# haoheliu/AudioLDM2

Measured on NVIDIA H100. Metric: 10s clips/sec @200 DDIM steps (audioldm2-full), higher is better.
Workload: dtype f16x2 (split-fp16 tensor-core operands: weights hi + lo, activations hi + lo in the convolutions and one plane on the token side; fp32 accumulate, fp32 residual stream)

## Files before the change

### audioldm2_b200/_lib.py

```python
from __future__ import annotations

import ctypes as C
import os
import shutil
import subprocess
import sys

HERE = os.path.dirname(os.path.abspath(__file__))
ROOT = os.path.dirname(HERE)
CSRC = os.path.join(HERE, "csrc")
LIB_PATH = os.path.join(HERE, "libaldm_b200.so")
SOURCES = ["gemm.cu", "prep.cu", "attention.cu", "elementwise.cu", "stft.cu", "program.cu", "engine_abi.cu", "microbench.cu",
           "cond/seqgen.cu"]
NVCC_FLAGS = ["-gencode", "arch=compute_90a,code=sm_90a", "-lineinfo", "-O3", "-std=c++17",
              "-Xcompiler", "-fPIC", "--use_fast_math=false"]

NVCC = shutil.which("nvcc") or os.path.join(os.environ.get("CUDA_HOME", "/usr/local/cuda"), "bin", "nvcc")

MAX_TAPS = 16
ABI_VERSION = 9

GEMM_TC, GEMM_SIMT, GEMM_TC_V1 = 0, 1, 2
GEMM_STATIC_B = 1 << 16
ACT_NONE, ACT_GEGLU, ACT_TANH, ACT_SILU, ACT_GELU_TANH = 0, 1, 2, 3, 4
OUT_F32, OUT_PLANES, OUT_NCHW, OUT_QKV = 0, 1, 2, 3
EPI_FAST, EPI_GEGLU, EPI_GENERIC, EPI_F32N, EPI_PLN = 0, 1, 2, 3, 4
RED_NONE, RED_REDUCE4, RED_GENERIC = 0, 1, 2
STORE_ROW, STORE_COMPACT, STORE_PAIR_PLN, STORE_PAIR_GEGLU, STORE_PAIR_QK = 0, 1, 2, 3, 4
PREP_COPY, PREP_SILU, PREP_LRELU, PREP_GN, PREP_GN_SILU, PREP_LN = 0, 1, 2, 3, 4, 5
OP_GEMM, OP_PREP, OP_ATTN, OP_SOFTMAX, OP_TEMB, OP_TRANSPOSE, OP_PACKB, OP_COPY = 1, 2, 3, 4, 5, 6, 7, 8
OP_SEQ_ASSEMBLE, OP_KV_ATTN, OP_SEQ_FEEDBACK = 9, 10, 11


class GemmDesc(C.Structure):
    _fields_ = [
        ("a_hi", C.c_void_p), ("a_lo", C.c_void_p), ("w_packed", C.c_void_p), ("w_plain", C.c_void_p),
        ("bias", C.c_void_p), ("rowvec", C.c_void_p), ("res", C.c_void_p), ("out", C.c_void_p),
        ("out_hi", C.c_void_p), ("out_lo", C.c_void_p), ("out2_hi", C.c_void_p), ("out2_lo", C.c_void_p),
        ("ws", C.c_void_p),
        ("B", C.c_int32), ("H", C.c_int32), ("W", C.c_int32), ("Cp", C.c_int32),
        ("up", C.c_int32), ("bmod", C.c_int32),
        ("OH", C.c_int32), ("OW", C.c_int32), ("sy", C.c_int32), ("sx", C.c_int32),
        ("ntaps", C.c_int32),
        ("dy", C.c_int16 * MAX_TAPS), ("dx", C.c_int16 * MAX_TAPS),
        ("N", C.c_int32), ("K", C.c_int32), ("Kpad", C.c_int32), ("bn", C.c_int32),
        ("ldo", C.c_int32), ("ld_res", C.c_int32), ("ld_rowvec", C.c_int32),
        ("OHF", C.c_int32), ("OWF", C.c_int32), ("osy", C.c_int32), ("ooy", C.c_int32),
        ("act", C.c_int32), ("out_mode", C.c_int32), ("accumulate", C.c_int32), ("splitk", C.c_int32),
        ("impl", C.c_int32), ("n_split", C.c_int32), ("tok_per_batch", C.c_int32), ("ld_t", C.c_int32),
        ("alpha", C.c_float),
    ]


class PrepDesc(C.Structure):
    _fields_ = [
        ("src0", C.c_void_p), ("src1", C.c_void_p), ("gamma", C.c_void_p), ("beta", C.c_void_p),
        ("out_hi", C.c_void_p), ("out_lo", C.c_void_p), ("scratch", C.c_void_p),
        ("rows", C.c_int32), ("c0", C.c_int32), ("c1", C.c_int32), ("Cp", C.c_int32),
        ("B", C.c_int32), ("HW", C.c_int32), ("groups", C.c_int32), ("mode", C.c_int32),
        ("eps", C.c_float), ("slope", C.c_float), ("src_nchw", C.c_int32),
    ]
# ... 93 lines not shown
        objs.append(o)
        cmd = [NVCC] + [f for f in NVCC_FLAGS if not f.startswith("--use_fast_math")] + ["-c", s, "-o", o]
        if verbose:
            print(" ".join(cmd))
        procs.append((cmd, subprocess.Popen(cmd, stdout=subprocess.PIPE, stderr=subprocess.STDOUT)))
    for cmd, p in procs:
        out, _ = p.communicate()
        if p.returncode != 0:
            raise RuntimeError("nvcc failed: %s\n%s" % (" ".join(cmd), out.decode()))
        if verbose and out:
            print(out.decode())
    cmd = [NVCC, "-shared", "-o", LIB_PATH] + objs + ["-lcudart"]
    r = subprocess.run(cmd, stdout=subprocess.PIPE, stderr=subprocess.STDOUT)
    if r.returncode != 0:
        raise RuntimeError("link failed: %s\n%s" % (" ".join(cmd), r.stdout.decode()))
    return LIB_PATH


_lib = None


def lib() -> C.CDLL:
    global _lib
    if _lib is not None:
        return _lib
    if not os.path.exists(LIB_PATH):
        raise RuntimeError(f"{LIB_PATH} is missing: run `python -c 'import __graft_entry__ as g; g.build()'`. "
                           "There is no CPU/PyTorch fallback for the native path.")
    L = C.CDLL(LIB_PATH)
    vp, i32, i64, f32 = C.c_void_p, C.c_int32, C.c_int64, C.c_float
    sig = {
        "aldm_gemm": (i32, [C.POINTER(GemmDesc), vp]),
        "aldm_gemm_variant": (i32, [C.POINTER(GemmDesc), C.POINTER(i32)]),
        "aldm_prep": (i32, [C.POINTER(PrepDesc), vp]),
        "aldm_pack_b": (i32, [vp, i32, i32, i32, i32, i32, vp, vp, vp]),
        "aldm_attention": (i32, [C.POINTER(AttnDesc), vp]),
        "aldm_kv_attention": (i32, [C.POINTER(KvAttnDesc), vp]),
        "aldm_seq_assemble": (i32, [C.POINTER(SeqAssembleDesc), vp]),
        "aldm_seq_feedback": (i32, [C.POINTER(SeqFeedbackDesc), vp]),
        "aldm_softmax_rows": (i32, [vp, i32, i32, f32, vp, vp, vp]),
        "aldm_timestep_embedding": (i32, [vp, i32, i32, vp, vp, vp, vp]),
        "aldm_ddim_step": (i32, [vp, vp, vp, vp, vp, vp, i64, f32, f32, f32, f32, f32, vp]),
        "aldm_masked_blend": (i32, [vp, vp, vp, vp, i32, i32, i32, f32, f32, vp]),
        "aldm_transpose_chw": (i32, [vp, vp, i32, i32, i32, i32, vp]),
        "aldm_posterior_sample": (i32, [vp, vp, vp, i32, i32, i32, f32, vp]),
        "aldm_stft_mel": (i32, [vp, i32, i32, i32, i32, vp, i32, vp, i32, vp]),
        "aldm_program_create": (i32, [C.POINTER(Op), i32, C.POINTER(vp)]),
        "aldm_program_run": (i32, [vp, vp]),
        "aldm_program_run_range": (i32, [vp, i32, i32, vp]),
        "aldm_program_capture": (i32, [vp, vp]),
        "aldm_program_replay": (i32, [vp, vp]),
        "aldm_program_num_launches": (i32, [vp]),
        "aldm_program_is_captured": (i32, [vp]),
        "aldm_program_destroy": (None, [vp]),
        "aldm_engine_create": (i32, [C.POINTER(EngineDesc), C.POINTER(vp)]),
        "aldm_engine_destroy": (None, [vp]),
        "aldm_engine_set_conditioning": (i32, [vp, i32, vp, vp, i32, vp, vp, i32, vp, vp]),
        "aldm_engine_precompute": (i32, [vp, vp]),
        "aldm_engine_unet_eps": (i32, [vp, vp, i64, vp, vp, vp]),
        "aldm_engine_ddim_step": (i32, [vp, vp, i64, vp, f32, f32, f32, f32, f32, vp, vp, vp]),
        "aldm_engine_vae_decode": (i32, [vp, vp, vp, vp]),
        "aldm_engine_vocoder": (i32, [vp, vp, vp, vp]),
        "aldm_engine_vae_encode": (i32, [vp, vp, vp, vp]),
        "aldm_sizeof_engine_desc": (C.c_size_t, []),
        "aldm_abi_version": (i32, []),
        "aldm_sizeof_op": (C.c_size_t, []),
        "aldm_sizeof_gemm_desc": (C.c_size_t, []),
        "aldm_offsetof_gemm": (C.c_size_t, [i32]),
        "aldm_last_error": (C.c_char_p, []),
        "aldm_device_check": (i32, [i32]),
        "aldm_debug_timeline": (i32, [vp, i32]),
        "aldm_debug_store_rate": (i32, [i32, i32, i32, i64, vp]),
    }
    for name, (res, args) in sig.items():
        fn = getattr(L, name)
        fn.restype = res
        fn.argtypes = args
    if L.aldm_abi_version() != ABI_VERSION:
        raise RuntimeError("libaldm_b200.so ABI version mismatch: rebuild")
    if L.aldm_sizeof_engine_desc() != C.sizeof(EngineDesc):
        raise RuntimeError("ctypes mirror of aldm_engine_desc does not match the C layout")
    if L.aldm_sizeof_op() != C.sizeof(Op) or L.aldm_sizeof_gemm_desc() != C.sizeof(GemmDesc):
        raise RuntimeError("ctypes mirror of aldm_op / aldm_gemm_desc does not match the C layout")
    _lib = L
    return L


EXPORTED = ["aldm_gemm", "aldm_gemm_variant", "aldm_prep", "aldm_pack_b", "aldm_attention", "aldm_softmax_rows",
            "aldm_kv_attention", "aldm_seq_assemble", "aldm_seq_feedback",
            "aldm_timestep_embedding", "aldm_ddim_step", "aldm_masked_blend", "aldm_transpose_chw",
            "aldm_posterior_sample", "aldm_stft_mel", "aldm_program_create", "aldm_program_run",
            "aldm_program_run_range", "aldm_program_capture", "aldm_program_replay",
            "aldm_program_num_launches", "aldm_program_is_captured", "aldm_program_destroy", "aldm_engine_create",
            "aldm_engine_destroy", "aldm_engine_set_conditioning", "aldm_engine_precompute", "aldm_engine_unet_eps",
            "aldm_engine_ddim_step", "aldm_engine_vae_decode", "aldm_engine_vocoder", "aldm_engine_vae_encode",
            "aldm_sizeof_engine_desc", "aldm_abi_version", "aldm_sizeof_op",
            "aldm_sizeof_gemm_desc", "aldm_offsetof_gemm", "aldm_last_error", "aldm_device_check", "aldm_debug_timeline",
            "aldm_debug_store_rate"]


def gemm_variant(d: GemmDesc) -> tuple:
    out = (C.c_int32 * 5)()
    check(lib().aldm_gemm_variant(C.byref(d), out), "gemm_variant")
    return tuple(out)


def check(rc: int, what: str = ""):
    if rc != 0:
        msg = lib().aldm_last_error().decode(errors="replace")
        raise RuntimeError(f"aldm error {rc} {what}: {msg}")


if __name__ == "__main__":
    print(build(verbose="-v" in sys.argv, force="-f" in sys.argv))
```

### audioldm2_b200/csrc/gemm.cu

```cuda
#include <stdlib.h>

#include "common.cuh"

namespace aldm {

struct RowInfo {
  int m, b, oh, ow;
  bool valid;
  long long orow;
};

__device__ __forceinline__ RowInfo decode_row(const aldm_gemm_desc& d, int m, int M) {
  RowInfo r;
  r.m = m;
  r.valid = m < M;
  int mm = r.valid ? m : 0;
  r.ow = mm % d.OW;
  int t = mm / d.OW;
  r.oh = t % d.OH;
  r.b = t / d.OH;
  r.orow = ((long long)r.b * d.OHF + (long long)r.oh * d.osy + d.ooy) * d.OWF + r.ow;
  return r;
}

// ... 203 lines not shown
    const auto o = cr.orow[it] * d.ldo + n;
    if (!PLANES_ONLY) *reinterpret_cast<float4*>(d.out + o) = x;
    if (PLANES_ONLY || d.out_hi) {
      uint2 h, l;
      split2(x.x, x.y, h.x, l.x);
      split2(x.z, x.w, h.y, l.y);
      *reinterpret_cast<uint2*>(reinterpret_cast<aldm_plane_t*>(d.out_hi) + o) = h;
      if (d.out_lo) *reinterpret_cast<uint2*>(reinterpret_cast<aldm_plane_t*>(d.out_lo) + o) = l;
    }
  }
  __syncwarp();
}

__device__ __forceinline__ void line_put_hi(uint8_t* tile, int lane, int part, const float* v) {
  uint8_t* wr = tile + lane * 128;
  const int sw = lane & 7;
#pragma unroll
  for (int j = 0; j < 4; ++j) *reinterpret_cast<uint4*>(wr + (((part * 4 + j) ^ sw) << 4)) = pack8_hi(v + 8 * j);
}
template <typename CR>
__device__ __forceinline__ void line_store_hi(const aldm_gemm_desc& d, const CR& cr, int n_group0, const uint8_t* tile, int lane) {
  __syncwarp();
  const int rs = lane >> 3, c8 = lane & 7;
  aldm_plane_t* out = reinterpret_cast<aldm_plane_t*>(d.out_hi);
#pragma unroll
  for (int it = 0; it < 8; ++it) {
    const int rr = it * 4 + rs;
    const uint4 x = *reinterpret_cast<const uint4*>(tile + rr * 128 + ((c8 ^ (rr & 7)) << 4));
    if ((cr.vmask >> rr) & 1u) *reinterpret_cast<uint4*>(out + (cr.orow[it] * d.ldo + n_group0 + c8 * 8)) = x;
  }
  __syncwarp();
}

template <int BN, int AP>
struct Tc3Cfg {
  static constexpr int BM = 128;
  static constexpr int BK = 64;
  static constexpr int A_BYTES = BM * 128;
  static constexpr int B_BYTES = BN * 128;
  static constexpr int STAGE_BYTES = AP * A_BYTES + 2 * B_BYTES;
  static constexpr int B_OFF = AP * A_BYTES;
  static constexpr int ACC_BYTES = BM * BN * 4;
  static constexpr int STG_BYTES = 4 * 32 * 33 * 4;
  static constexpr int SMEM_MAX = 227 * 1024;
  static constexpr int FIT = (SMEM_MAX - 1024 - 256 - STG_BYTES - ACC_BYTES) / STAGE_BYTES;
  static constexpr int STAGES = FIT > 4 ? 4 : FIT;
  static constexpr int SMEM_BYTES = STAGES * STAGE_BYTES + ACC_BYTES + 1024  + 256  + STG_BYTES;
  static_assert(STAGES >= 2, "pipeline needs two stages");
  static_assert(SMEM_BYTES <= SMEM_MAX, "shared memory");
};

template <int BN>
__device__ __forceinline__ void acc_st_frag(float* accb, int row0, int lane, const float* d) {
  const int g = lane >> 2, t = lane & 3;
#pragma unroll
  for (int h = 0; h < 2; ++h) {
    const int row = row0 + g + 8 * h;
    float* rp = accb + row * BN + 2 * (t & 1);
#pragma unroll
    for (int j = 0; j < BN / 8; ++j)
      *reinterpret_cast<float2*>(rp + (((2 * j + (t >> 1)) ^ (row & 7)) << 2)) = make_float2(d[4 * j + 2 * h], d[4 * j + 2 * h + 1]);
  }
}
template <int BN>
__device__ __forceinline__ void acc_ld32(const float* accb, int row, int c0, uint32_t* r) {
  const float* rp = accb + row * BN;
#pragma unroll
  for (int j = 0; j < 8; ++j) {
    const float4 x = *reinterpret_cast<const float4*>(rp + ((((c0 >> 2) + j) ^ (row & 7)) << 2));
    r[4 * j] = __float_as_uint(x.x); r[4 * j + 1] = __float_as_uint(x.y);
    r[4 * j + 2] = __float_as_uint(x.z); r[4 * j + 3] = __float_as_uint(x.w);
  }
}
constexpr int kProdRegs = 80, kConsRegs = 136, kEpiRegs = 160;
static_assert(kProdRegs + 2 * kConsRegs + kEpiRegs == 4 * 128, "register split must use exactly the launch allocation");
template <int R>
__device__ __forceinline__ void setmaxnreg_dec() { asm volatile("setmaxnreg.dec.sync.aligned.u32 %0;" ::"n"(R)); }
template <int R>
__device__ __forceinline__ void setmaxnreg_inc() { asm volatile("setmaxnreg.inc.sync.aligned.u32 %0;" ::"n"(R)); }

__device__ long long g_timeline[4 * 256 * 2];
#define ALDM_TL(role, i, ph)                                                      \
  do {                                                                            \
    if ((dbg & 128) && blockIdx.x == 0 && (i) < 256) g_timeline[((role) * 256 + (i)) * 2 + (ph)] = clock64(); \
  } while (0)

enum { EPI_FAST = ALDM_EPI_FAST, EPI_GEGLU = ALDM_EPI_GEGLU, EPI_GENERIC = ALDM_EPI_GENERIC, EPI_F32N = ALDM_EPI_F32N,
       EPI_PLN = ALDM_EPI_PLN };

struct FastDiv {
  unsigned long long M;
  int sh;
  int d;
  __device__ __forceinline__ int div(int n) const {
    return (int)(((unsigned long long)(unsigned)n * M) >> sh);
  }
  __device__ __forceinline__ void divmod(int n, int& q, int& r) const { q = div(n); r = n - q * d; }
};
static FastDiv make_fastdiv(int d) {
  FastDiv f;
  int l = 0;
  while ((1ll << l) < d) ++l;
  f.M = (unsigned long long)((((unsigned __int128)1) << (32 + l)) / (unsigned)d) + 1ull;
  f.sh = 32 + l;
  f.d = d;
  if (d == 1) { f.M = 1ull << 32; f.sh = 32; }
  return f;
}
struct Tc3Divs {
  FastDiv ow, oh, cp, tn, bmod;
  int plain;
  int store;
};

template <int BN, int EPI, int AP>
__global__ void __launch_bounds__(512, 1) gemm_tc3_kernel(const __grid_constant__ aldm_gemm_desc d, int tiles_m, int tiles_n,
                                                           const __grid_constant__ Tc3Divs fd) {
  using C = Tc3Cfg<BN, AP>;
  extern __shared__ uint8_t smem_raw[];
  const uint32_t raw = smem_u32(smem_raw);
  const uint32_t base = (raw + 1023u) & ~1023u;
  const uint32_t acc_base = base + C::STAGES * C::STAGE_BYTES;
  const uint32_t bar_base = acc_base + C::ACC_BYTES;
  auto full_bar = [&](int s) { return bar_base + 8u * s; };
  auto empty_bar = [&](int s) { return bar_base + 8u * (C::STAGES + s); };
  const uint32_t acc_full = bar_base + 8u * (2 * C::STAGES);
  const uint32_t acc_empty = acc_full + 8u;
  float* accb = reinterpret_cast<float*>(smem_raw + (acc_base - raw));

  const int tid = threadIdx.x;
  const int warp = tid >> 5;
  const int lane = tid & 31;
  const int M = d.B * d.OH * d.OW;
  const int nkb_total = d.Kpad / C::BK;
  const int total = tiles_m * tiles_n * d.splitk;
  const int dbg = d.impl >> 8;

  if (tid == 0) {
    for (int s = 0; s < C::STAGES; ++s) {
      mbar_init(full_bar(s), 128 + 1);
      mbar_init(empty_bar(s), 8);
    }
    mbar_init(acc_full, 8);
    mbar_init(acc_empty, 4);
    fence_barrier_init();
  }
  __syncthreads();

  auto tile_coords = [&](int id, int& mt, int& nt, int& z, int& kb0, int& nkb) {
    int r = id;
    z = 0; kb0 = 0; nkb = nkb_total;
    if (d.splitk > 1) {
      z = id % d.splitk;
      r = id / d.splitk;
      kb0 = (int)(((long long)z * nkb_total) / d.splitk);
      nkb = (int)(((long long)(z + 1) * nkb_total) / d.splitk) - kb0;
    }
    fd.tn.divmod(r, mt, nt);
  };

  if (warp >= 8 && warp < 12) {
    setmaxnreg_dec<kProdRegs>();
    const int ptid = tid - 256;
    const int j = ptid & 7;
    const int rbase = ptid >> 3;
    const uint32_t swz = (uint32_t)((j ^ (rbase & 7)) << 4);
    const int Hs = d.H >> d.up, Ws = d.W >> d.up;
    const aldm_plane_t* ahi = reinterpret_cast<const aldm_plane_t*>(d.a_hi);
    const aldm_plane_t* alo = reinterpret_cast<const aldm_plane_t*>(d.a_lo);
    uint32_t cnt = 0;
    int last_mt = -1;
    int rowoff[8];
    uint32_t tapmask[8];
    uint32_t yx0[8];
    auto decode_rows = [&](int mt) {
#pragma unroll
      for (int i = 0; i < 8; ++i) {
        const int m = mt * C::BM + rbase + 16 * i;
        uint32_t msk = 0, yx = 0;
        int off = 0;
        if (fd.plain) {
          if (m < M) { msk = 16u; off = m * d.Cp; }
        } else if (m < M) {
          int t, ow, b, oh;
          fd.ow.divmod(m, t, ow);
          fd.oh.divmod(t, b, oh);
          const int y0 = oh * d.sy, x0 = ow * d.sx;
          int bs = b;
          if (d.bmod > 0) { int q; fd.bmod.divmod(b, q, bs); }
          const int pb = bs * Hs;
          yx = (uint32_t)y0 | ((uint32_t)x0 << 16);
          for (int tp = 0; tp < d.ntaps; ++tp) {
            const int ih = y0 + d.dy[tp], iw = x0 + d.dx[tp];
            if (ih >= 0 && ih < d.H && iw >= 0 && iw < d.W) msk |= 16u << tp;
          }
// ... 69 lines not shown
          if (!(dbg & 1)) {
#define ALDM_A_ROW(i)                                                                            \
            {                                                                                      \
              const uint32_t nb = (tapmask[i] >> sh) & 16u;                                        \
              cp_async_16_off<(i) * 2048>(sa2, ab + rowoff[i], nb);                                \
              if (AP == 2) cp_async_16_off<(i) * 2048 + C::A_BYTES>(sa2, abl + rowoff[i], nb);     \
            }
            ALDM_A_ROW(0) ALDM_A_ROW(1) ALDM_A_ROW(2) ALDM_A_ROW(3) ALDM_A_ROW(4) ALDM_A_ROW(5) ALDM_A_ROW(6) ALDM_A_ROW(7)
#undef ALDM_A_ROW
          }
        } else {
          const int dy = d.dy[tp], dx = d.dx[tp];
#pragma unroll
          for (int i = 0; i < 8; ++i) {
            const bool ok = kvalid && ((tapmask[i] >> (tp + 4)) & 1u);
            long long off = 0;
            const int ih = (int)(yx0[i] & 0xffffu) + dy, iw = (int)(yx0[i] >> 16) + dx;
            if (ok) off = ((long long)(rowoff[i] + (ih >> 1)) * Ws + (iw >> 1)) * d.Cp + c;
            const uint32_t dst = sa + (uint32_t)(rbase + 16 * i) * 128u;
            cp_async_16(dst, ahi + off, ok ? 16u : 0u);
            if (AP == 2) cp_async_16(dst + C::A_BYTES, alo + off, ok ? 16u : 0u);
          }
        }
        cp_async_mbar_arrive_noinc(full_bar(s));
        if (ptid == 0) ALDM_TL(0, cnt, 1);
        c += C::BK;
        while (c >= d.Cp) { c -= d.Cp; ++tap; }
      }
    }
  } else if (warp < 8) {
    setmaxnreg_inc<kConsRegs>();
    pdl_wait();
    const int wg = warp >> 2;
    uint32_t cnt = 0, tl = 0;
    float acc[BN / 2];
    for (int id = blockIdx.x; id < total; id += gridDim.x, ++tl) {
      int mt, nt, z, kb0, nkb;
      tile_coords(id, mt, nt, z, kb0, nkb);
#pragma unroll
      for (int i = 0; i < BN / 2; ++i) acc[i] = 0.f;
      for (int it = 0; it < nkb; ++it, ++cnt) {
        const int s = cnt % C::STAGES;
        if (it > 0) {
          wgmma_wait<0>();
          if (lane == 0) mbar_arrive(empty_bar((cnt - 1) % C::STAGES));
        }
        mbar_wait(full_bar(s), (cnt / C::STAGES) & 1);
        if (tid == 0) ALDM_TL(2, cnt, 0);
        fence_proxy_async();
        const uint32_t sa = base + s * C::STAGE_BYTES;
        const uint64_t da_hi = wgmma_desc_sw128(sa + wg * 64 * 128);
        const uint64_t da_lo = wgmma_desc_sw128(sa + C::A_BYTES + wg * 64 * 128);
        const uint64_t db_hi = wgmma_desc_sw128(sa + C::B_OFF);
        const uint64_t db_lo = wgmma_desc_sw128(sa + C::B_OFF + C::B_BYTES);
        wgmma_fence();
        if (!(dbg & 4)) {
#pragma unroll
          for (int ks = 0; ks < 4; ++ks) {
            const uint64_t o = (uint64_t)(ks * 2);
            wgmma_ss<BN>(acc, da_hi + o, db_lo + o, 1);
            if (AP == 2) wgmma_ss<BN>(acc, da_lo + o, db_hi + o, 1);
            wgmma_ss<BN>(acc, da_hi + o, db_hi + o, 1);
          }
        }
        wgmma_commit();
        if (tid == 0) ALDM_TL(2, cnt, 1);
      }
      wgmma_wait<0>();
      wgmma_fence_regs<BN / 2>(acc);
      if (lane == 0) mbar_arrive(empty_bar((cnt - 1) % C::STAGES));
      if (tid == 0 && id + (int)gridDim.x >= total) pdl_launch();
      mbar_wait(acc_empty, (tl & 1) ^ 1);
      acc_st_frag<BN>(accb, wg * 64 + (warp & 3) * 16, lane, acc);
      __syncwarp();
      if (lane == 0) mbar_arrive(acc_full);
    }
  } else {
    setmaxnreg_inc<kEpiRegs>();
    pdl_wait();
    const int ew = warp - 12;
    const int trow_in_tile = ew * 32 + lane;
    float* stg = reinterpret_cast<float*>(smem_raw + (bar_base + 256 - raw)) + ew * (32 * 33);
    uint8_t* stg8 = reinterpret_cast<uint8_t*>(stg);
    constexpr bool kCompact = EPI == EPI_F32N || EPI == EPI_PLN;
    constexpr int NCH = BN / 32;
    constexpr int NRV = NCH > 1 ? 2 : 1;
    constexpr int NGV = BN >= 64 ? BN / 64 : 1;
    const bool pair_pln = EPI == EPI_PLN && BN >= 64 && fd.store == ALDM_STORE_PAIR_PLN;
    const bool pair_geglu = EPI == EPI_GEGLU && BN == 128 && fd.store == ALDM_STORE_PAIR_GEGLU;
    const bool pair_qk = EPI == EPI_FAST && BN >= 64 && fd.store == ALDM_STORE_PAIR_QK;
    const bool has_res = kCompact && d.res != nullptr;
    uint32_t tl = 0;
    for (int id = blockIdx.x; id < total; id += gridDim.x, ++tl) {
      int mt, nt, z, kb0, nkb;
      tile_coords(id, mt, nt, z, kb0, nkb);
      const int m = mt * C::BM + trow_in_tile;
      RowInfo r;
      {
        r.m = m; r.valid = m < M;
        const int mm = r.valid ? m : 0;
        int t;
        fd.ow.divmod(mm, t, r.ow);
        fd.oh.divmod(t, r.b, r.oh);
        r.orow = ((long long)r.b * d.OHF + (long long)r.oh * d.osy + d.ooy) * d.OWF + r.ow;
      }
      CoRows cr;
      CoRows32 cr32;
      if (kCompact) cr32 = co_rows32(r, lane); else cr = co_rows(r, lane);
      float4 pb4[NCH], prv[NRV][8];
      if (kCompact) {
#pragma unroll
        for (int ch = 0; ch < NCH; ++ch) {
          const int n = nt * BN + 32 * ch + (lane & 7) * 4;
          pb4[ch] = (d.bias && n < d.N) ? __ldg(reinterpret_cast<const float4*>(d.bias + n)) : make_float4(0.f, 0.f, 0.f, 0.f);
        }
#pragma unroll
        for (int ch = 0; ch < NRV; ++ch)
          if (has_res) co_load_res32(d, cr32, nt * BN + 32 * ch, d.N, lane, prv[ch]);
      }
      float pln_b[NCH];
#pragma unroll
      for (int ch = 0; ch < NCH; ++ch) {
        const int n = nt * BN + 32 * ch + lane;
        pln_b[ch] = (pair_pln && d.bias && n < d.N) ? __ldg(d.bias + n) : 0.f;
      }
      float gb_v[NGV], gb_g[NGV];
#pragma unroll
      for (int c = 0; c < NGV; ++c) {
        gb_v[c] = 0.f; gb_g[c] = 0.f;
        if (EPI == EPI_GEGLU && d.bias && d.splitk == 1) {
          gb_v[c] = __ldg(d.bias + nt * BN + 32 * c + lane);
// ... 239 lines not shown
      pc0 = tile * d.bn + sub * 32; n0 = tile * (d.bn / 2) + sub * 32; n_out = d.N / 2;
    } else {
      pc0 = ch * 32; n0 = pc0; n_out = d.N;
    }
    const float* wv = d.w_plain + (long long)(pc0 + lane) * d.Kpad;
    const float* wg = wv + (long long)(d.bn / 2) * d.Kpad;
    float acc = 0.f, accg = 0.f;
    for (int tap = 0; tap < d.ntaps; ++tap) {
      const int ih = r.oh * d.sy + d.dy[tap], iw = r.ow * d.sx + d.dx[tap];
      if (ih < 0 || ih >= d.H || iw < 0 || iw >= d.W) continue;
      const long long off = ((long long)(bsrc * Hs + (ih >> d.up)) * Ws + (iw >> d.up)) * d.Cp;
      const float* wt = wv + tap * d.Cp;
      const float* wgt = wg + tap * d.Cp;
      for (int c = 0; c < d.Cp; ++c) {
        const float a = plane_to_f(ahi[off + c]) + (alo ? plane_to_f(alo[off + c]) : 0.f);
        acc = fmaf(a, __ldg(wt + c), acc);
        if (geglu) accg = fmaf(a, __ldg(wgt + c), accg);
      }
    }
    float v[32], g[32];
#pragma unroll
    for (int i = 0; i < 32; ++i) {
      v[i] = __shfl_sync(0xffffffffu, acc, i);
      g[i] = __shfl_sync(0xffffffffu, accg, i);
    }
    if (lane == 0) {
      epi_activate(d, r, pc0, v, g);
      epi_finish(d, r, n0, 32, v, n_out);
    }
  }
}

struct GemmVariant {
  int bn, epi, ap, red, store;
};

static GemmVariant gemm_select(const aldm_gemm_desc& d) {
  GemmVariant v{d.bn, EPI_GENERIC, d.a_lo ? 2 : 1, ALDM_RED_NONE, ALDM_STORE_ROW};
  const int BN = d.bn;
  const bool geglu = d.act == ALDM_ACT_GEGLU;
  const int n_out = geglu ? d.N / 2 : d.N;
  const bool co = d.splitk == 1 && n_out % 4 == 0 && d.ldo % 4 == 0 && (!d.res || d.ld_res % 4 == 0) &&
                  (d.out_mode == ALDM_OUT_F32 || d.out_mode == ALDM_OUT_PLANES || d.out_mode == ALDM_OUT_QKV);
  const long long out_rows = (long long)d.B * d.OHF * d.OWF;
  const int ld_max = d.ldo > d.ld_res ? d.ldo : d.ld_res;
  static const bool compact_on = [] { const char* e = getenv("ALDM_EPI_COMPACT"); return !(e && e[0] == '0'); }();
  const bool plain = compact_on && co && d.act == ALDM_ACT_NONE && d.alpha == 1.0f && !d.accumulate && !d.rowvec &&
                     out_rows * ld_max < (1ll << 31) &&
                     (!d.bias || aligned16(d.bias)) && (!d.res || aligned16(d.res));
  if (co && geglu && !d.res && d.out_mode != ALDM_OUT_QKV && BN >= 64) v.epi = EPI_GEGLU;
  else if (plain && d.out_mode == ALDM_OUT_F32 && aligned16(d.out) && (!d.out_hi || d.ldo % 4 == 0)) v.epi = EPI_F32N;
  else if (plain && d.out_mode == ALDM_OUT_PLANES) v.epi = EPI_PLN;
  else if (co && d.act == ALDM_ACT_NONE) v.epi = EPI_FAST;
  if (v.epi == EPI_F32N || v.epi == EPI_PLN) v.store = ALDM_STORE_COMPACT;
  const bool pair_ok = d.out_lo == nullptr && d.splitk == 1 && d.ldo % 8 == 0 && aligned16(d.out_hi);
  if (v.epi == EPI_PLN && BN >= 64 && pair_ok && d.res == nullptr && d.N % BN == 0) v.store = ALDM_STORE_PAIR_PLN;
  if (v.epi == EPI_GEGLU && BN == 128 && pair_ok && d.out_mode == ALDM_OUT_PLANES && (d.N / 2) % 64 == 0) v.store = ALDM_STORE_PAIR_GEGLU;
  if (v.epi == EPI_FAST && BN >= 64 && pair_ok && d.out_mode == ALDM_OUT_QKV && d.res == nullptr && d.n_split % 64 == 0)
    v.store = ALDM_STORE_PAIR_QK;
  if (d.splitk > 1) {
    const bool fast = d.act == ALDM_ACT_NONE && d.alpha == 1.0f && !d.accumulate && d.N % 4 == 0 && d.ldo % 4 == 0 &&
                      (d.out_mode == ALDM_OUT_F32 || d.out_mode == ALDM_OUT_PLANES) && (!d.res || (d.ld_res % 4 == 0 && aligned16(d.res))) &&
                      (!d.bias || aligned16(d.bias)) && (!d.rowvec || (d.ld_rowvec % 4 == 0 && aligned16(d.rowvec))) &&
                      (d.out_mode != ALDM_OUT_F32 || aligned16(d.out));
    v.red = fast ? ALDM_RED_REDUCE4 : ALDM_RED_GENERIC;
  }
  return v;
}

template <int BN, int EPI, int AP>
static int launch_tc3_ap(const aldm_gemm_desc& d, int M, const GemmVariant& v, cudaStream_t st) {
  using C = Tc3Cfg<BN, AP>;
  static bool configured = false;
  if (!configured) {
    ALDM_CHECK_CUDA(cudaFuncSetAttribute(gemm_tc3_kernel<BN, EPI, AP>, cudaFuncAttributeMaxDynamicSharedMemorySize, C::SMEM_BYTES));
    configured = true;
  }
  const int tiles_m = cdiv(M, C::BM), tiles_n = cdiv(d.N, BN);
  const long long total = (long long)tiles_m * tiles_n * d.splitk;
  const int grid = (int)(total < num_sms() ? total : num_sms());
  Tc3Divs fd;
  fd.ow = make_fastdiv(d.OW); fd.oh = make_fastdiv(d.OH); fd.cp = make_fastdiv(d.Cp); fd.tn = make_fastdiv(tiles_n);
  fd.bmod = make_fastdiv(d.bmod > 0 ? d.bmod : 1);
  fd.plain = d.ntaps == 1 && d.dy[0] == 0 && d.dx[0] == 0 && d.sy == 1 && d.sx == 1 && d.up == 0 && d.bmod <= 0 &&
             d.OH == d.H && d.OW == d.W;
  fd.store = v.store;
  ALDM_CHECK_CUDA(launch_pdl(gemm_tc3_kernel<BN, EPI, AP>, dim3(grid), dim3(512), C::SMEM_BYTES, st, d, tiles_m, tiles_n, fd));
  ALDM_CHECK_CUDA(cudaGetLastError());
  if (d.splitk > 1) {
    const int Mpad = tiles_m * C::BM, Npad = tiles_n * BN;
    const int chunks = (d.act == ALDM_ACT_GEGLU) ? (Npad / BN) * (BN / 64) : Npad / 32;
    const long long tot = (long long)M * chunks;
    if (v.red == ALDM_RED_REDUCE4) {
      const long long q = (long long)M * ((d.N + 3) / 4);
      splitk_reduce4_kernel<<<(unsigned)((q + 255) / 256), 256, 0, st>>>(d, Mpad, Npad);
    } else {
      splitk_epilogue_kernel<<<(unsigned)((tot + 127) / 128), 128, 0, st>>>(d, Mpad, Npad);
    }
    ALDM_CHECK_CUDA(cudaGetLastError());
  }
  return ALDM_OK;
}

template <int BN, int EPI>
static int launch_tc3_epi(const aldm_gemm_desc& d, int M, const GemmVariant& v, cudaStream_t st) {
  return v.ap == 2 ? launch_tc3_ap<BN, EPI, 2>(d, M, v, st) : launch_tc3_ap<BN, EPI, 1>(d, M, v, st);
}

template <int BN>
static int launch_tc2(const aldm_gemm_desc& d, int M, const GemmVariant& v, cudaStream_t st) {
  switch (v.epi) {
    case EPI_GEGLU: return launch_tc3_epi<BN, EPI_GEGLU>(d, M, v, st);
    case EPI_F32N: return launch_tc3_epi<BN, EPI_F32N>(d, M, v, st);
    case EPI_PLN: return launch_tc3_epi<BN, EPI_PLN>(d, M, v, st);
    case EPI_FAST: return launch_tc3_epi<BN, EPI_FAST>(d, M, v, st);
    default: return launch_tc3_epi<BN, EPI_GENERIC>(d, M, v, st);
  }
}

int gemm_num_launches(const aldm_gemm_desc& d) { return ((d.impl & 0xff) != ALDM_GEMM_SIMT && d.splitk > 1) ? 2 : 1; }

static int gemm_check(const aldm_gemm_desc& d) {
  const long long Mll = (long long)d.B * d.OH * d.OW;
  ALDM_REQUIRE(Mll > 0 && Mll < (1ll << 31), ALDM_E_SHAPE, "gemm: bad M=%lld", Mll);
  ALDM_REQUIRE(d.bn == 32 || d.bn == 64 || d.bn == 128, ALDM_E_UNSUPPORTED, "gemm: bn=%d unsupported", d.bn);
  ALDM_REQUIRE(d.Cp % 8 == 0 && d.Cp > 0, ALDM_E_SHAPE, "gemm: Cp=%d must be a positive multiple of 8", d.Cp);
  ALDM_REQUIRE(d.ntaps >= 1 && d.ntaps <= ALDM_MAX_TAPS, ALDM_E_SHAPE, "gemm: ntaps=%d", d.ntaps);
  ALDM_REQUIRE(d.K == d.ntaps * d.Cp, ALDM_E_SHAPE, "gemm: K=%d != ntaps*Cp=%d", d.K, d.ntaps * d.Cp);
  ALDM_REQUIRE(d.Kpad % 64 == 0 && d.Kpad >= d.K, ALDM_E_SHAPE, "gemm: Kpad=%d (K=%d)", d.Kpad, d.K);
  ALDM_REQUIRE(d.N >= 1, ALDM_E_SHAPE, "gemm: N=%d", d.N);
  ALDM_REQUIRE(d.a_hi, ALDM_E_ARG, "gemm: null A plane");
  ALDM_REQUIRE(aligned16(d.a_hi) && aligned16(d.a_lo), ALDM_E_ALIGN, "gemm: A planes not 16B aligned");
  ALDM_REQUIRE(d.up == 0 || d.up == 1, ALDM_E_ARG, "gemm: up=%d", d.up);
  ALDM_REQUIRE(d.up == 0 || (d.H < 65536 && d.W < 65536), ALDM_E_SHAPE, "gemm: upsampled input %dx%d too large", d.H, d.W);
// ... 36 lines not shown
    ALDM_CHECK_CUDA(cudaGetLastError());
    return ALDM_OK;
  }
  const GemmVariant v = gemm_select(d);
  switch (v.bn) {
    case 128: return launch_tc2<128>(d, M, v, st);
    case 64: return launch_tc2<64>(d, M, v, st);
    default: return launch_tc2<32>(d, M, v, st);
  }
}

}

extern "C" int aldm_debug_timeline(long long* host_out, int32_t n) {
  using namespace aldm;
  ALDM_REQUIRE(host_out && n > 0 && n <= 4 * 256 * 2, ALDM_E_ARG, "debug_timeline: bad arguments");
  ALDM_CHECK_CUDA(cudaMemcpyFromSymbol(host_out, g_timeline, sizeof(long long) * n));
  void* sym = nullptr;
  ALDM_CHECK_CUDA(cudaGetSymbolAddress(&sym, g_timeline));
  ALDM_CHECK_CUDA(cudaMemset(sym, 0, sizeof(g_timeline)));
  return ALDM_OK;
}

extern "C" int aldm_gemm_variant(const aldm_gemm_desc* d, int32_t out[5]) {
  if (!d || !out) { aldm::set_error("aldm_gemm_variant: null argument"); return ALDM_E_ARG; }
  const int rc = aldm::gemm_check(*d);
  if (rc) return rc;
  if ((d->impl & 0xff) == ALDM_GEMM_SIMT) { aldm::set_error("aldm_gemm_variant: the SIMT checker has no variants"); return ALDM_E_UNSUPPORTED; }
  const aldm::GemmVariant v = aldm::gemm_select(*d);
  out[0] = v.bn; out[1] = v.epi; out[2] = v.ap; out[3] = v.red; out[4] = v.store;
  return ALDM_OK;
}

extern "C" int aldm_gemm(const aldm_gemm_desc* d, void* stream) {
  if (!d) { aldm::set_error("aldm_gemm: null desc"); return ALDM_E_ARG; }
  return aldm::gemm_launch(*d, reinterpret_cast<cudaStream_t>(stream));
}
```

### include/aldm_b200.h

```cpp
#ifndef ALDM_B200_H_
#define ALDM_B200_H_

#include <stdint.h>
#include <stddef.h>

#ifdef __cplusplus
extern "C" {
#endif

#define ALDM_ABI_VERSION 9
#define ALDM_MAX_TAPS 16

enum {
  ALDM_OK = 0,
  ALDM_E_ARG = -1,
  ALDM_E_SHAPE = -2,
  ALDM_E_ALIGN = -3,
  ALDM_E_CUDA = -4,
  ALDM_E_NOMEM = -5,
  ALDM_E_UNSUPPORTED = -6
};


enum { ALDM_GEMM_TC = 0, ALDM_GEMM_SIMT = 1, ALDM_GEMM_TC_V1 = 2 };
// ... 5 lines not shown
  const void* a_hi;
  const void* a_lo;
  const void* w_packed;
  const float* w_plain;
  const float* bias;
  const float* rowvec;
  const float* res;
  float* out;
  void* out_hi;
  void* out_lo;
  void* out2_hi;
  void* out2_lo;
  float* ws;
  int32_t B, H, W, Cp;
  int32_t up, bmod;
  int32_t OH, OW, sy, sx;
  int32_t ntaps;
  int16_t dy[ALDM_MAX_TAPS];
  int16_t dx[ALDM_MAX_TAPS];
  int32_t N, K, Kpad, bn;
  int32_t ldo, ld_res, ld_rowvec;
  int32_t OHF, OWF, osy, ooy;
  int32_t act, out_mode, accumulate, splitk, impl;
  int32_t n_split, tok_per_batch, ld_t;
  float alpha;
} aldm_gemm_desc;

int aldm_gemm(const aldm_gemm_desc* d, void* stream);

enum { ALDM_EPI_FAST = 0, ALDM_EPI_GEGLU = 1, ALDM_EPI_GENERIC = 2, ALDM_EPI_F32N = 3, ALDM_EPI_PLN = 4 };
enum { ALDM_RED_NONE = 0, ALDM_RED_REDUCE4 = 1, ALDM_RED_GENERIC = 2 };
enum { ALDM_STORE_ROW = 0, ALDM_STORE_COMPACT = 1, ALDM_STORE_PAIR_PLN = 2, ALDM_STORE_PAIR_GEGLU = 3, ALDM_STORE_PAIR_QK = 4 };
int aldm_gemm_variant(const aldm_gemm_desc* d, int32_t out[5]);


enum { ALDM_PREP_COPY = 0, ALDM_PREP_SILU = 1, ALDM_PREP_LRELU = 2,
       ALDM_PREP_GN = 3, ALDM_PREP_GN_SILU = 4, ALDM_PREP_LN = 5 };

typedef struct aldm_prep_desc {
  const float* src0; const float* src1;
  const float* gamma; const float* beta;
  void* out_hi; void* out_lo;
  double* scratch;
  int32_t rows, c0, c1, Cp;
  int32_t B, HW, groups;
  int32_t mode;
  float eps, slope;
  int32_t src_nchw;
} aldm_prep_desc;

int aldm_prep(const aldm_prep_desc* d, void* stream);

int aldm_pack_b(const float* src, int32_t lds, int32_t transpose, int32_t N, int32_t K,
                int32_t bn, void* dst_packed, float* dst_plain, void* stream);


typedef struct aldm_attn_desc {
  const void* q_hi; const void* q_lo; const void* k_hi; const void* k_lo; const void* vt_hi; const void* vt_lo;
  const float* mask;
  void* out_hi; void* out_lo;
  int32_t B, heads, Nq, Nk, ldq, ldk, ld_t, ldo, q_col, k_col, kv_bmod, impl;
  float scale;
} aldm_attn_desc;

int aldm_attention(const aldm_attn_desc* d, void* stream);

// ... 157 lines not shown
```

Baseline: 1.783.

## Add halo-slab A loading for 3x3 stride-1 convolutions in the TC GEMM

Adds a halo mode to the warp-specialized implicit-GEMM kernel for 3x3 stride-1 same-size convolutions. Each CTA loads one 2D spatial tile plus a one-pixel halo per 64-channel block into a double-buffered shared slab, and the nine taps reuse it through shifted wgmma descriptors instead of gathering A separately for every tap. This cuts redundant global and L2 reads of activations, but forces BN=64, gives up A pipeline stages for slab space, and serializes wgmma waits per tap. The mode is on by default and can be turned off with ALDM_CONV_HALO=0.

```diff
diff --git a/audioldm2_b200/_lib.py b/audioldm2_b200/_lib.py
--- a/audioldm2_b200/_lib.py
+++ b/audioldm2_b200/_lib.py
@@ -27,6 +27,7 @@
 EPI_FAST, EPI_GEGLU, EPI_GENERIC, EPI_F32N, EPI_PLN = 0, 1, 2, 3, 4
 RED_NONE, RED_REDUCE4, RED_GENERIC = 0, 1, 2
 STORE_ROW, STORE_COMPACT, STORE_PAIR_PLN, STORE_PAIR_GEGLU, STORE_PAIR_QK = 0, 1, 2, 3, 4
+AMODE_GATHER, AMODE_HALO = 0, 1
 PREP_COPY, PREP_SILU, PREP_LRELU, PREP_GN, PREP_GN_SILU, PREP_LN = 0, 1, 2, 3, 4, 5
 OP_GEMM, OP_PREP, OP_ATTN, OP_SOFTMAX, OP_TEMB, OP_TRANSPOSE, OP_PACKB, OP_COPY = 1, 2, 3, 4, 5, 6, 7, 8
 OP_SEQ_ASSEMBLE, OP_KV_ATTN, OP_SEQ_FEEDBACK = 9, 10, 11
@@ -186,6 +187,7 @@
     sig = {
         "aldm_gemm": (i32, [C.POINTER(GemmDesc), vp]),
         "aldm_gemm_variant": (i32, [C.POINTER(GemmDesc), C.POINTER(i32)]),
+        "aldm_gemm_a_mode": (i32, [C.POINTER(GemmDesc), C.POINTER(i32)]),
         "aldm_prep": (i32, [C.POINTER(PrepDesc), vp]),
         "aldm_pack_b": (i32, [vp, i32, i32, i32, i32, i32, vp, vp, vp]),
         "aldm_attention": (i32, [C.POINTER(AttnDesc), vp]),
@@ -240,7 +242,7 @@
     return L
 
 
-EXPORTED = ["aldm_gemm", "aldm_gemm_variant", "aldm_prep", "aldm_pack_b", "aldm_attention", "aldm_softmax_rows",
+EXPORTED = ["aldm_gemm", "aldm_gemm_variant", "aldm_gemm_a_mode", "aldm_prep", "aldm_pack_b", "aldm_attention", "aldm_softmax_rows",
             "aldm_kv_attention", "aldm_seq_assemble", "aldm_seq_feedback",
             "aldm_timestep_embedding", "aldm_ddim_step", "aldm_masked_blend", "aldm_transpose_chw",
             "aldm_posterior_sample", "aldm_stft_mel", "aldm_program_create", "aldm_program_run",
@@ -259,6 +261,12 @@
     return tuple(out)
 
 
+def gemm_a_mode(d: GemmDesc) -> int:
+    out = C.c_int32()
+    check(lib().aldm_gemm_a_mode(C.byref(d), C.byref(out)), "gemm_a_mode")
+    return out.value
+
+
 def check(rc: int, what: str = ""):
     if rc != 0:
         msg = lib().aldm_last_error().decode(errors="replace")
diff --git a/audioldm2_b200/csrc/gemm.cu b/audioldm2_b200/csrc/gemm.cu
--- a/audioldm2_b200/csrc/gemm.cu
+++ b/audioldm2_b200/csrc/gemm.cu
@@ -259,30 +259,36 @@
   __syncwarp();
 }
 
-template <int BN, int AP>
+template <int BN, int AP, int HALO = 0>
 struct Tc3Cfg {
   static constexpr int BM = 128;
   static constexpr int BK = 64;
   static constexpr int A_BYTES = BM * 128;
   static constexpr int B_BYTES = BN * 128;
-  static constexpr int STAGE_BYTES = AP * A_BYTES + 2 * B_BYTES;
-  static constexpr int B_OFF = AP * A_BYTES;
+  static constexpr int HALO_PIX = 180;
+  static constexpr int SLAB_PLANE = HALO ? (HALO_PIX * 128 + 1023) / 1024 * 1024 : 0;
+  static constexpr int NSLAB = HALO ? 2 : 0;
+  static constexpr int SLAB_SET = AP * SLAB_PLANE;
+  static constexpr int SLAB_BYTES = NSLAB * SLAB_SET;
+  static constexpr int STAGE_BYTES = (HALO ? 0 : AP * A_BYTES) + 2 * B_BYTES;
+  static constexpr int B_OFF = HALO ? 0 : AP * A_BYTES;
   static constexpr int ACC_BYTES = BM * BN * 4;
   static constexpr int STG_BYTES = 4 * 32 * 33 * 4;
   static constexpr int SMEM_MAX = 227 * 1024;
-  static constexpr int FIT = (SMEM_MAX - 1024 - 256 - STG_BYTES - ACC_BYTES) / STAGE_BYTES;
+  static constexpr int FIT = (SMEM_MAX - 1024 - 256 - STG_BYTES - ACC_BYTES - SLAB_BYTES) / STAGE_BYTES;
   static constexpr int STAGES = FIT > 4 ? 4 : FIT;
-  static constexpr int SMEM_BYTES = STAGES * STAGE_BYTES + ACC_BYTES + 1024  + 256  + STG_BYTES;
+  static constexpr int SMEM_BYTES = SLAB_BYTES + STAGES * STAGE_BYTES + ACC_BYTES + 1024  + 256  + STG_BYTES;
   static_assert(STAGES >= 2, "pipeline needs two stages");
   static_assert(SMEM_BYTES <= SMEM_MAX, "shared memory");
+  static_assert(!HALO || BN == 64, "the halo path is built for BN = 64");
 };
 
 template <int BN>
-__device__ __forceinline__ void acc_st_frag(float* accb, int row0, int lane, const float* d) {
+__device__ __forceinline__ void acc_st_frag(float* accb, int row0, int hstep, int lane, const float* d) {
   const int g = lane >> 2, t = lane & 3;
 #pragma unroll
   for (int h = 0; h < 2; ++h) {
-    const int row = row0 + g + 8 * h;
+    const int row = row0 + g + hstep * h;
     float* rp = accb + row * BN + 2 * (t & 1);
 #pragma unroll
     for (int j = 0; j < BN / 8; ++j)
@@ -301,6 +307,10 @@
 }
 constexpr int kProdRegs = 80, kConsRegs = 136, kEpiRegs = 160;
 static_assert(kProdRegs + 2 * kConsRegs + kEpiRegs == 4 * 128, "register split must use exactly the launch allocation");
+__device__ __forceinline__ uint64_t wgmma_desc_sw128_sbo(uint32_t smem_addr, uint32_t sbo) {
+  return static_cast<uint64_t>((smem_addr >> 4) & 0x3FFFu) | (1ull << 16) | (static_cast<uint64_t>((sbo >> 4) & 0x3FFFu) << 32) |
+         (1ull << 62);
+}
 template <int R>
 __device__ __forceinline__ void setmaxnreg_dec() { asm volatile("setmaxnreg.dec.sync.aligned.u32 %0;" ::"n"(R)); }
 template <int R>
@@ -338,21 +348,27 @@
   FastDiv ow, oh, cp, tn, bmod;
   int plain;
   int store;
+  FastDiv tpi, tx;
+  int tw_sh;
 };
 
-template <int BN, int EPI, int AP>
+template <int BN, int EPI, int AP, int HALO>
 __global__ void __launch_bounds__(512, 1) gemm_tc3_kernel(const __grid_constant__ aldm_gemm_desc d, int tiles_m, int tiles_n,
                                                            const __grid_constant__ Tc3Divs fd) {
-  using C = Tc3Cfg<BN, AP>;
+  using C = Tc3Cfg<BN, AP, HALO>;
   extern __shared__ uint8_t smem_raw[];
   const uint32_t raw = smem_u32(smem_raw);
   const uint32_t base = (raw + 1023u) & ~1023u;
-  const uint32_t acc_base = base + C::STAGES * C::STAGE_BYTES;
+  const uint32_t slab = base;
+  auto stage_base = [&](int s) { return base + C::SLAB_BYTES + s * C::STAGE_BYTES; };
+  const uint32_t acc_base = base + C::SLAB_BYTES + C::STAGES * C::STAGE_BYTES;
   const uint32_t bar_base = acc_base + C::ACC_BYTES;
   auto full_bar = [&](int s) { return bar_base + 8u * s; };
   auto empty_bar = [&](int s) { return bar_base + 8u * (C::STAGES + s); };
   const uint32_t acc_full = bar_base + 8u * (2 * C::STAGES);
   const uint32_t acc_empty = acc_full + 8u;
+  auto slab_full = [&](int i) { return acc_empty + 8u + 8u * i; };
+  auto slab_empty = [&](int i) { return acc_empty + 8u + 8u * (C::NSLAB + i); };
   float* accb = reinterpret_cast<float*>(smem_raw + (acc_base - raw));
 
   const int tid = threadIdx.x;
@@ -365,11 +381,15 @@
 
   if (tid == 0) {
     for (int s = 0; s < C::STAGES; ++s) {
-      mbar_init(full_bar(s), 128 + 1);
+      mbar_init(full_bar(s), HALO ? 1 : 128 + 1);
       mbar_init(empty_bar(s), 8);
     }
     mbar_init(acc_full, 8);
     mbar_init(acc_empty, 4);
+    for (int i = 0; i < C::NSLAB; ++i) {
+      mbar_init(slab_full(i), 96);
+      mbar_init(slab_empty(i), 8);
+    }
     fence_barrier_init();
   }
   __syncthreads();
@@ -388,6 +408,91 @@
 
   if (warp >= 8 && warp < 12) {
     setmaxnreg_dec<kProdRegs>();
+    if constexpr (HALO) {
+      const int ncb = d.Cp >> 6;
+      const int tw = 1 << fd.tw_sh, th = C::BM >> fd.tw_sh, hw = tw + 2;
+      if (warp == 11) {
+        if (!(d.impl & ALDM_GEMM_STATIC_B)) pdl_wait();
+        if (elect_one()) {
+          uint32_t cnt = 0;
+          for (int id = blockIdx.x; id < total; id += gridDim.x) {
+            int mt, nt, z, kb0, nkb;
+            tile_coords(id, mt, nt, z, kb0, nkb);
+            const int per = d.bn / BN;
+            const long long wtile = 2ll * d.bn * 128;
+            const uint8_t* wsrc = reinterpret_cast<const uint8_t*>(d.w_packed) + (long long)(nt / per) * nkb_total * wtile +
+                                  (nt % per) * C::B_BYTES;
+            for (int cb = 0; cb < ncb; ++cb)
+              for (int tap = 0; tap < 9; ++tap, ++cnt) {
+                const int s = cnt % C::STAGES;
+                mbar_wait(empty_bar(s), ((cnt / C::STAGES) & 1) ^ 1);
+                if (dbg & 2) { mbar_arrive(full_bar(s)); continue; }
+                const uint8_t* src = wsrc + (long long)(tap * ncb + cb) * wtile;
+                mbar_arrive_expect_tx(full_bar(s), 2 * C::B_BYTES);
+                bulk_g2s(stage_base(s), src, C::B_BYTES, full_bar(s));
+                bulk_g2s(stage_base(s) + C::B_BYTES, src + wtile / 2, C::B_BYTES, full_bar(s));
+              }
+          }
+        }
+        return;
+      }
+      const int pt = tid - 256;
+      const int j = pt & 7, hr0 = pt >> 3;
+      const int Ws = d.W >> d.up;
+      int relc[15];
+      uint32_t e_top = 0, e_bot = 0, e_lft = 0, e_rgt = 0;
+#pragma unroll
+      for (int i = 0; i < 15; ++i) {
+        const int hr = hr0 + 12 * i, hy = hr / hw, hx = hr - hy * hw;
+        relc[i] = (((hy - 1) >> d.up) * Ws + ((hx - 1) >> d.up)) * d.Cp;
+        e_top |= (uint32_t)(hy == 0) << i;
+        e_bot |= (uint32_t)(hy == th + 1) << i;
+        e_lft |= (uint32_t)(hx == 0) << i;
+        e_rgt |= (uint32_t)(hx == tw + 1) << i;
+      }
+      const uint32_t d_even = slab + hr0 * 128 + ((j ^ (hr0 & 7)) << 4);
+      const uint32_t d_odd = slab + hr0 * 128 + ((j ^ ((hr0 + 4) & 7)) << 4);
+      const aldm_plane_t* ahi = reinterpret_cast<const aldm_plane_t*>(d.a_hi);
+      const aldm_plane_t* alo = reinterpret_cast<const aldm_plane_t*>(d.a_lo);
+      uint32_t cnt = 0;
+      pdl_wait();
+      for (int id = blockIdx.x; id < total; id += gridDim.x) {
+        int mt, nt, z, kb0, nkb, b, t, ty, tx;
+        tile_coords(id, mt, nt, z, kb0, nkb);
+        fd.tpi.divmod(mt, b, t);
+        fd.tx.divmod(t, ty, tx);
+        const int y0 = ty * th, x0 = tx * tw;
+        int bs = b;
+        if (d.bmod > 0) { int q; fd.bmod.divmod(b, q, bs); }
+        uint32_t valid = 0x7fffu;
+        if (y0 == 0) valid &= ~e_top;
+        if (y0 + th == d.H) valid &= ~e_bot;
+        if (x0 == 0) valid &= ~e_lft;
+        if (x0 + tw == d.W) valid &= ~e_rgt;
+        const long long pix0 = ((long long)(bs * (d.H >> d.up) + (y0 >> d.up)) * Ws + (x0 >> d.up)) * d.Cp + j * 8;
+        for (int cb = 0; cb < ncb; ++cb, ++cnt) {
+          const int sl = cnt % C::NSLAB;
+          mbar_wait(slab_empty(sl), ((cnt / C::NSLAB) & 1) ^ 1);
+          const uint32_t de = d_even + sl * C::SLAB_SET, dod = d_odd + sl * C::SLAB_SET;
+          if (!(dbg & 1)) {
+            const aldm_plane_t* ab = ahi + pix0 + cb * 64;
+            const aldm_plane_t* abl = alo + pix0 + cb * 64;
+#define ALDM_HALO_PIX(i)                                                                                   \
+            {                                                                                                \
+              const uint32_t nb = ((valid >> (i)) & 1u) << 4;                                                \
+              cp_async_16_off<(i) * 1536>((i) & 1 ? dod : de, ab + relc[i], nb);                             \
+              if (AP == 2) cp_async_16_off<(i) * 1536 + C::SLAB_PLANE>((i) & 1 ? dod : de, abl + relc[i], nb); \
+            }
+            ALDM_HALO_PIX(0) ALDM_HALO_PIX(1) ALDM_HALO_PIX(2) ALDM_HALO_PIX(3) ALDM_HALO_PIX(4) ALDM_HALO_PIX(5)
+            ALDM_HALO_PIX(6) ALDM_HALO_PIX(7) ALDM_HALO_PIX(8) ALDM_HALO_PIX(9) ALDM_HALO_PIX(10) ALDM_HALO_PIX(11)
+            ALDM_HALO_PIX(12) ALDM_HALO_PIX(13) ALDM_HALO_PIX(14)
+#undef ALDM_HALO_PIX
+          }
+          cp_async_mbar_arrive_noinc(slab_full(sl));
+        }
+      }
+      return;
+    }
     const int ptid = tid - 256;
     const int j = ptid & 7;
     const int rbase = ptid >> 3;
@@ -523,6 +628,62 @@
     setmaxnreg_inc<kConsRegs>();
     pdl_wait();
     const int wg = warp >> 2;
+    if constexpr (HALO) {
+      const int ncb = d.Cp >> 6;
+      const int tw = 1 << fd.tw_sh, hw = tw + 2;
+      const int row_c = (tw == 8 ? 8 * wg + 1 : 1) * hw + (tw == 16 ? 8 * wg : 0) + 1;
+      const uint32_t sbo = (uint32_t)hw * 128u;
+      uint32_t cnt = 0, scnt = 0, tl = 0;
+      float acc[BN / 2];
+      for (int id = blockIdx.x; id < total; id += gridDim.x, ++tl) {
+#pragma unroll
+        for (int i = 0; i < BN / 2; ++i) acc[i] = 0.f;
+        for (int cb = 0; cb < ncb; ++cb, ++scnt) {
+          const int sl = scnt % C::NSLAB;
+          if (cb > 0) {
+            wgmma_wait<0>();
+            if (lane == 0) { mbar_arrive(empty_bar((cnt - 1) % C::STAGES)); mbar_arrive(slab_empty((scnt - 1) % C::NSLAB)); }
+          }
+          mbar_wait(slab_full(sl), (scnt / C::NSLAB) & 1);
+          fence_proxy_async();
+#pragma unroll 1
+          for (int tap = 0; tap < 9; ++tap, ++cnt) {
+            const int s = cnt % C::STAGES;
+            if (tap > 0) {
+              wgmma_wait<0>();
+              if (lane == 0) mbar_arrive(empty_bar((cnt - 1) % C::STAGES));
+            }
+            mbar_wait(full_bar(s), (cnt / C::STAGES) & 1);
+            const uint32_t sa = slab + sl * C::SLAB_SET + (uint32_t)(row_c + d.dy[tap] * hw + d.dx[tap]) * 128u;
+            const uint64_t da_hi = wgmma_desc_sw128_sbo(sa, sbo);
+            const uint64_t da_lo = wgmma_desc_sw128_sbo(sa + C::SLAB_PLANE, sbo);
+            const uint64_t db_hi = wgmma_desc_sw128(stage_base(s));
+            const uint64_t db_lo = wgmma_desc_sw128(stage_base(s) + C::B_BYTES);
+            wgmma_fence();
+            if (!(dbg & 4)) {
+#pragma unroll
+              for (int ks = 0; ks < 4; ++ks) {
+                const uint64_t o = (uint64_t)(ks * 2);
+                wgmma_ss<BN>(acc, da_hi + o, db_lo + o, 1);
+                if (AP == 2) wgmma_ss<BN>(acc, da_lo + o, db_hi + o, 1);
+                wgmma_ss<BN>(acc, da_hi + o, db_hi + o, 1);
+              }
+            }
+            wgmma_commit();
+          }
+        }
+        wgmma_wait<0>();
+        wgmma_fence_regs<BN / 2>(acc);
+        if (lane == 0) { mbar_arrive(empty_bar((cnt - 1) % C::STAGES)); mbar_arrive(slab_empty((scnt - 1) % C::NSLAB)); }
+        if (tid == 0 && id + (int)gridDim.x >= total) pdl_launch();
+        mbar_wait(acc_empty, (tl & 1) ^ 1);
+        if (tw == 16) acc_st_frag<BN>(accb, 32 * (warp & 3) + 8 * wg, 16, lane, acc);
+        else acc_st_frag<BN>(accb, wg * 64 + (warp & 3) * 16, 8, lane, acc);
+        __syncwarp();
+        if (lane == 0) mbar_arrive(acc_full);
+      }
+      return;
+    }
     uint32_t cnt = 0, tl = 0;
     float acc[BN / 2];
     for (int id = blockIdx.x; id < total; id += gridDim.x, ++tl) {
@@ -562,7 +723,7 @@
       if (lane == 0) mbar_arrive(empty_bar((cnt - 1) % C::STAGES));
       if (tid == 0 && id + (int)gridDim.x >= total) pdl_launch();
       mbar_wait(acc_empty, (tl & 1) ^ 1);
-      acc_st_frag<BN>(accb, wg * 64 + (warp & 3) * 16, lane, acc);
+      acc_st_frag<BN>(accb, wg * 64 + (warp & 3) * 16, 8, lane, acc);
       __syncwarp();
       if (lane == 0) mbar_arrive(acc_full);
     }
@@ -587,7 +748,16 @@
       tile_coords(id, mt, nt, z, kb0, nkb);
       const int m = mt * C::BM + trow_in_tile;
       RowInfo r;
-      {
+      if (HALO) {
+        int t, ty, tx;
+        fd.tpi.divmod(mt, r.b, t);
+        fd.tx.divmod(t, ty, tx);
+        r.oh = ty * (C::BM >> fd.tw_sh) + (trow_in_tile >> fd.tw_sh);
+        r.ow = (tx << fd.tw_sh) + (trow_in_tile & ((1 << fd.tw_sh) - 1));
+        r.m = (r.b * d.OH + r.oh) * d.OW + r.ow;
+        r.valid = true;
+        r.orow = ((long long)r.b * d.OHF + (long long)r.oh * d.osy + d.ooy) * d.OWF + r.ow;
+      } else {
         r.m = m; r.valid = m < M;
         const int mm = r.valid ? m : 0;
         int t;
@@ -893,12 +1063,23 @@
 }
 
 struct GemmVariant {
-  int bn, epi, ap, red, store;
+  int bn, epi, ap, red, store, amode;
 };
 
+static bool halo_ok(const aldm_gemm_desc& d) {
+  static const bool on = [] { const char* e = getenv("ALDM_CONV_HALO"); return !(e && e[0] == '0'); }();
+  if (!on || (d.bn != 64 && d.bn != 128) || d.act == ALDM_ACT_GEGLU || d.splitk != 1 || d.ntaps != 9 || d.sy != 1 ||
+      d.sx != 1 || d.Cp % 64 != 0 || d.OH != d.H || d.OW != d.W)
+    return false;
+  for (int t = 0; t < d.ntaps; ++t)
+    if (d.dy[t] < -1 || d.dy[t] > 1 || d.dx[t] < -1 || d.dx[t] > 1) return false;
+  return (d.W % 16 == 0 && d.H % 8 == 0) || (d.W == 8 && d.H % 16 == 0);
+}
+
 static GemmVariant gemm_select(const aldm_gemm_desc& d) {
-  GemmVariant v{d.bn, EPI_GENERIC, d.a_lo ? 2 : 1, ALDM_RED_NONE, ALDM_STORE_ROW};
-  const int BN = d.bn;
+  const bool halo = halo_ok(d);
+  GemmVariant v{halo ? 64 : d.bn, EPI_GENERIC, d.a_lo ? 2 : 1, ALDM_RED_NONE, ALDM_STORE_ROW, halo ? ALDM_AMODE_HALO : ALDM_AMODE_GATHER};
+  const int BN = v.bn;
   const bool geglu = d.act == ALDM_ACT_GEGLU;
   const int n_out = geglu ? d.N / 2 : d.N;
   const bool co = d.splitk == 1 && n_out % 4 == 0 && d.ldo % 4 == 0 && (!d.res || d.ld_res % 4 == 0) &&
@@ -929,12 +1110,12 @@
   return v;
 }
 
-template <int BN, int EPI, int AP>
-static int launch_tc3_ap(const aldm_gemm_desc& d, int M, const GemmVariant& v, cudaStream_t st) {
-  using C = Tc3Cfg<BN, AP>;
+template <int BN, int EPI, int AP, int HALO>
+static int launch_tc3_mode(const aldm_gemm_desc& d, int M, const GemmVariant& v, cudaStream_t st) {
+  using C = Tc3Cfg<BN, AP, HALO>;
   static bool configured = false;
   if (!configured) {
-    ALDM_CHECK_CUDA(cudaFuncSetAttribute(gemm_tc3_kernel<BN, EPI, AP>, cudaFuncAttributeMaxDynamicSharedMemorySize, C::SMEM_BYTES));
+    ALDM_CHECK_CUDA(cudaFuncSetAttribute(gemm_tc3_kernel<BN, EPI, AP, HALO>, cudaFuncAttributeMaxDynamicSharedMemorySize, C::SMEM_BYTES));
     configured = true;
   }
   const int tiles_m = cdiv(M, C::BM), tiles_n = cdiv(d.N, BN);
@@ -946,7 +1127,11 @@
   fd.plain = d.ntaps == 1 && d.dy[0] == 0 && d.dx[0] == 0 && d.sy == 1 && d.sx == 1 && d.up == 0 && d.bmod <= 0 &&
              d.OH == d.H && d.OW == d.W;
   fd.store = v.store;
-  ALDM_CHECK_CUDA(launch_pdl(gemm_tc3_kernel<BN, EPI, AP>, dim3(grid), dim3(512), C::SMEM_BYTES, st, d, tiles_m, tiles_n, fd));
+  fd.tw_sh = d.W == 8 ? 3 : 4;
+  const int tw = 1 << fd.tw_sh, th = C::BM / tw;
+  fd.tx = make_fastdiv(HALO ? d.W / tw : 1);
+  fd.tpi = make_fastdiv(HALO ? (d.H / th) * (d.W / tw) : 1);
+  ALDM_CHECK_CUDA(launch_pdl(gemm_tc3_kernel<BN, EPI, AP, HALO>, dim3(grid), dim3(512), C::SMEM_BYTES, st, d, tiles_m, tiles_n, fd));
   ALDM_CHECK_CUDA(cudaGetLastError());
   if (d.splitk > 1) {
     const int Mpad = tiles_m * C::BM, Npad = tiles_n * BN;
@@ -961,6 +1146,13 @@
     ALDM_CHECK_CUDA(cudaGetLastError());
   }
   return ALDM_OK;
+}
+
+template <int BN, int EPI, int AP>
+static int launch_tc3_ap(const aldm_gemm_desc& d, int M, const GemmVariant& v, cudaStream_t st) {
+  if constexpr (BN == 64)
+    if (v.amode == ALDM_AMODE_HALO) return launch_tc3_mode<BN, EPI, AP, 1>(d, M, v, st);
+  return launch_tc3_mode<BN, EPI, AP, 0>(d, M, v, st);
 }
 
 template <int BN, int EPI>
@@ -1063,6 +1255,15 @@
   return ALDM_OK;
 }
 
+extern "C" int aldm_gemm_a_mode(const aldm_gemm_desc* d, int32_t* mode) {
+  if (!d || !mode) { aldm::set_error("aldm_gemm_a_mode: null argument"); return ALDM_E_ARG; }
+  const int rc = aldm::gemm_check(*d);
+  if (rc) return rc;
+  if ((d->impl & 0xff) == ALDM_GEMM_SIMT) { aldm::set_error("aldm_gemm_a_mode: the SIMT checker has no variants"); return ALDM_E_UNSUPPORTED; }
+  *mode = aldm::gemm_select(*d).amode;
+  return ALDM_OK;
+}
+
 extern "C" int aldm_gemm(const aldm_gemm_desc* d, void* stream) {
   if (!d) { aldm::set_error("aldm_gemm: null desc"); return ALDM_E_ARG; }
   return aldm::gemm_launch(*d, reinterpret_cast<cudaStream_t>(stream));
diff --git a/include/aldm_b200.h b/include/aldm_b200.h
--- a/include/aldm_b200.h
+++ b/include/aldm_b200.h
@@ -61,6 +61,8 @@
 enum { ALDM_RED_NONE = 0, ALDM_RED_REDUCE4 = 1, ALDM_RED_GENERIC = 2 };
 enum { ALDM_STORE_ROW = 0, ALDM_STORE_COMPACT = 1, ALDM_STORE_PAIR_PLN = 2, ALDM_STORE_PAIR_GEGLU = 3, ALDM_STORE_PAIR_QK = 4 };
 int aldm_gemm_variant(const aldm_gemm_desc* d, int32_t out[5]);
+enum { ALDM_AMODE_GATHER = 0, ALDM_AMODE_HALO = 1 };
+int aldm_gemm_a_mode(const aldm_gemm_desc* d, int32_t* mode);
 
 
 enum { ALDM_PREP_COPY = 0, ALDM_PREP_SILU = 1, ALDM_PREP_LRELU = 2,
```

Result: faster. 1.846, median of 6 (+3.5%).
